# Anony-CFFM/CFFM

Hardware: AMD Instinct MI355X
Metric: training examples/sec, frappe 10-field dim32; embedding-gather %HBM roofline (higher is better)
Workload: dtype f32; 1 GPU; frappe shape: synthetic libfm, 10 fields, 5382 features, inner/outer dim 32, batch 256 per GPU, selu, Adagrad lr 0.05, square_loss (README.md:28); global_batch=256, id_distribution=uniform, tables=replicated, parallelism=single

## Files before the change

cffm_amd/csrc/common.hpp:

```cpp
#pragma once
#include <hip/hip_runtime.h>
#include <stdint.h>

#include "../../include/cffm_hip.h"

#define CFFM_WAVE 64

#ifdef CFFM_PHASE_TIMERS
static __device__ unsigned long long cffm_phase_times[16];
static __device__ unsigned long long cffm_wg_times[2 * 1024];
static __device__ unsigned long long cffm_bwd_times[48];
#define PHASE_MARKB(i, wg) do { if ((wg) == 7 && threadIdx.x == 0) cffm_bwd_times[i] = wall_clock64(); } while (0)
#define PHASE_MARK(i) do { if (blockIdx.x == 7 && threadIdx.x == 0) cffm_phase_times[i] = wall_clock64(); } while (0)
#define PHASE_MARK2(i) do {} while (0)
#define PHASE_MARK3(i) do { if (CL && blockIdx.x == 7 && threadIdx.x == 0) cffm_phase_times[8 + (i)] = wall_clock64(); } while (0)
#else
#define PHASE_MARK(i) do {} while (0)
#define PHASE_MARK2(i) do {} while (0)
#define PHASE_MARK3(i) do {} while (0)
#define PHASE_MARKB(i, wg) do {} while (0)
#endif

typedef float f32x4 __attribute__((ext_vector_type(4)));
__device__ __forceinline__ int fused_c_off(int l, int c0, int c1, int D, int Pp) {
    if (l == 0) return c0;
    int o = c1;
    for (int k = 1; k < l; ++k) { const int S = D >> (k + 1); o += S * S * Pp * 4; }
    return o;
}


#define CFFM_CHECK_LAUNCH()                          \
    do {                                             \
        hipError_t e__ = hipGetLastError();          \
        if (e__ != hipSuccess) return (int)e__;      \
    } while (0)

static inline int ceil_div_i(int64_t a, int64_t b) { return (int)((a + b - 1) / b); }
static inline int ilog2_i(int v) { int r = 0; while ((1 << (r + 1)) <= v) ++r; return r; }
static inline int id_key_bits(int M) {
    int bits = 1;
    while ((1ll << bits) <= (long long)M && bits < 31) ++bits;
    return bits;
}

static constexpr int CFFM_LDS_SHARED_CU = 150 * 1024;
static constexpr int CFFM_LDS_WHOLE_CU = 160 * 1024 - 512;
template <class KernelT>
static inline int set_lds(KernelT k, size_t lds) {
    if (lds > 64 * 1024) {
        hipError_t e = hipFuncSetAttribute((const void*)k, hipFuncAttributeMaxDynamicSharedMemorySize, (int)lds);
        if (e != hipSuccess) return (int)e;
    }
// ... 97 lines not shown
#define CFFM_NSLAB_SMALL 256
static inline int small_slabs(int32_t B) { return B <= 256 ? 256 : (B >= 1024 ? 1024 : (B + 255) / 256 * 256); }
struct SlabRange { int64_t off, len, base; int nslab; };
struct SlabPlan {
    SlabRange r[CFFM_MAX_LAYERS + 3];
    int n;
    int64_t total;
    int head_front, inner, conv0, head_back;
};

static inline bool bwd_top_ok(const cffm_shape_t* s, int32_t B) {
    const int F = s->F, Pp = (F * (F - 1) / 2 + 15) / 16 * 16;
    const int live = ilog2_i(s->D) - 1;
    return Pp <= 64 && B <= 256 && s->inner_conv && s->outer_conv && live >= 2;
}
static inline int bwd_top_first_layer(const cffm_shape_t* s) {
    const int live = ilog2_i(s->D) - 1;
    return live - 2 >= 1 ? live - 2 : 1;
}
static inline int conv_slabs_plain(const cffm_shape_t* s, int32_t B, int l) {
    const int F = s->F, Pp = (F * (F - 1) / 2 + 15) / 16 * 16;
    const int64_t S = s->D >> (l + 1);
    return (Pp <= 64 && (int64_t)B * S * S >= 256 * 64) ? 256 : CFFM_NSLAB;
}
static inline bool conv_pair_slabs_ok(int Pp, int l, int64_t rows, int nslab) {
    return l >= 1 && Pp <= 64 && (rows + nslab - 1) / nslab < 128;
}
static inline bool conv_pair_ok(const cffm_shape_t* s, int32_t B, int l) {
    const int F = s->F, Pp = (F * (F - 1) / 2 + 15) / 16 * 16;
    const int64_t S = s->D >> (l + 1);
    return conv_pair_slabs_ok(Pp, l, (int64_t)B * S * S, conv_slabs_plain(s, B, l));
}
#define CFFM_TOP_SLAB_ROWS 32
static inline bool bwd_fused01_ok(const cffm_shape_t* s, int32_t B) {
    const int F = s->F, Pp = (F * (F - 1) / 2 + 15) / 16 * 16;
    return bwd_top_ok(s, B) && s->D == 32 && Pp <= 48 && B >= 64;
}
static inline bool top_wgrad_deferred(const cffm_shape_t* s, int32_t B) {
    return bwd_top_ok(s, B) && !bwd_fused01_ok(s, B) && conv_pair_ok(s, B, bwd_top_first_layer(s) - 1);
}
static inline int conv_slabs(const cffm_shape_t* s, int32_t B, int l) {
    const int64_t S = s->D >> (l + 1);
    if (bwd_fused01_ok(s, B)) {
        if (l <= 1) return 256;
        const int64_t n = ((int64_t)B * S * S + CFFM_TOP_SLAB_ROWS - 1) / CFFM_TOP_SLAB_ROWS;
        return n < 1 ? 1 : (int)n;
    }
    if (bwd_top_ok(s, B) && l >= bwd_top_first_layer(s)) {
        if (!top_wgrad_deferred(s, B)) return 256;
        const int64_t n = ((int64_t)B * S * S + 63) / 64;
        return n < 1 ? 1 : (n > 256 ? 256 : (int)n);
    }
    return conv_slabs_plain(s, B, l);
}

static inline void make_slab_plan(const cffm_shape_t* s, int32_t B, const cffm_theta_layout_t& tl, SlabPlan* p) {
    int n = 0;
    int64_t base = 0;
    auto add = [&](int64_t off, int64_t end, int nslab) {
        p->r[n].off = off; p->r[n].len = end - off; p->r[n].base = base; p->r[n].nslab = nslab;
        base += (end - off) * nslab;
        return n++;
    };
    const int64_t convs = tl.live > 0 ? tl.conv_w[0] : tl.d1_w;
    p->head_front = add(0, tl.inner_cw, small_slabs(B));
    p->inner = add(tl.inner_cw, convs, small_slabs(B));
    p->conv0 = n;
    for (int l = 0; l < tl.live; ++l)
        add(tl.conv_w[l], l + 1 < tl.live ? tl.conv_w[l + 1] : tl.d1_w, conv_slabs(s, B, l));
// ... 125 lines not shown
```

cffm_amd/csrc/conv.hip:

```cpp
#include <cstdlib>
#include <cstring>

#include "internal.hpp"

#include <type_traits>

#include <stdlib.h>
#include "inner_body.hpp"
#include "head_body.hpp"
#include "sort_body.hpp"

#define KSTEP 32
#define WG_KM 64

__device__ __forceinline__ int64_t xcd_tile(int64_t per_xcd) {
    const int64_t id = blockIdx.x;
    return (id & 7) * per_xcd + (id >> 3);
}
__host__ __device__ static inline int64_t xcd_per(int64_t tiles) { return (tiles + 7) / 8; }

struct RowPos { int b, y, x; };
__device__ __forceinline__ RowPos row_pos(int64_t m, int lgSo) {
    RowPos p;
    const int So = 1 << lgSo;
// ... 1597 lines not shown
        char* smem_i = smem + fa.early_off;
        if (fa.rank_keys) rank_keys_body<NW>(fa.ids, fa.n_rows, b, fa.inner.g.F, fa.inner.g.M, fa.keys_sorted, smem_i);
        PHASE_MARK(0);
        inner_fwd_body<ACT>(fa.inner, b, smem_i, early ? reinterpret_cast<float*>(smem + fa.es_off) : nullptr, fa.inner.g.D + 1, park);
        if (lds_act) lds_barrier(); else __syncthreads();
        PHASE_MARK(1);
        conv0_fact_fwd_body<NT, NW>(fa.conv[0], b, smem, CL(0), early);
        for (int l = 1; l < fa.live; ++l) {
            if (lds_act) lds_barrier(); else __syncthreads();
            PHASE_MARK(1 + l);
            const ConvArgs& ca = fa.conv[l];
            const int64_t rows = 1ll << (2 * ca.lgSo), m_lo = (int64_t)b * rows, m_hi = m_lo + rows;
            if (rows >= 64) {
                for (int64_t m0 = m_lo; m0 < m_hi; m0 += 64) {
                    if (m0 > m_lo) lds_barrier();
                    conv_fwd_taps_body<NT, 4 / G, false, G, ACT>(ca, m0, m_hi, smem, CL(l - 1), CL(l), m_lo);
                }
            } else if (rows >= 32) {
                conv_fwd_taps_body<NT, (G >= 2 ? 1 : 2), false, G, ACT>(ca, m_lo, m_hi, smem, CL(l - 1), CL(l), m_lo);
            } else {
                conv_fwd_taps_body<NT, 1, false, G, ACT>(ca, m_lo, m_hi, smem, CL(l - 1), CL(l), m_lo);
            }
        }
        if (lds_act) lds_barrier(); else __syncthreads();
        PHASE_MARK(1 + fa.live);
        head_fwd_body<NW, ACT>(fa.head, b, smem, lds_act, fa.c0_off, fa.c1_off);
        PHASE_MARK(2 + fa.live);
    }
#ifdef CFFM_PHASE_TIMERS
    if (threadIdx.x == 0) cffm_wg_times[2 * blockIdx.x + 1] = wall_clock64();
#endif
}

template <int NT, int F_, int D_, int NW>
__device__ __forceinline__ void conv0_fact_bwd_body(const DgradArgs& a, float* __restrict__ slabW, float* __restrict__ slabB,
                                                    int64_t slab_stride, char* smem, int wg, int nwg) {
    constexpr int PP = NT * 16, S = 16, NTH = 64 * NW, XQ = 16 / NW;
    const int F = F_ ? F_ : a.F, D = D_ ? D_ : a.D, Dp = D + 1, P = F_ ? F_ * (F_ - 1) / 2 : a.P, F2 = 2 * F;
    const int TP = S * PP + 16;
    float* Wl = reinterpret_cast<float*>(smem);
    float* T = Wl + 4 * PP * PP;
    float* part = T + 2 * F * TP;
    float* dEi = part + NW * 16 * 32;
    float* dEj = dEi + 32 * 16;
    float* bred = dEj + 32 * 16;
    float* rs = bred + NW * PP;
    float* Es = rs + 2 * F;
    const int tid = threadIdx.x, lane = tid & 63, wave = tid >> 6, r = lane & 15, kk = lane >> 4;
    float* sw = slabW + (int64_t)wg * slab_stride;
    float* sb = slabB + (int64_t)wg * slab_stride;
    PHASE_MARKB(12, wg);
    {
        const float4* wsrc = reinterpret_cast<const float4*>(a.W);
        for (int i = tid; i < 4 * PP * PP / 4; i += NTH) reinterpret_cast<float4*>(Wl)[i] = wsrc[i];
        for (int e = tid; e < 4 * (PP - P) * PP; e += NTH) {
            const int tap = e / ((PP - P) * PP), o = e - tap * ((PP - P) * PP);
            sw[(tap * PP + P) * PP + o] = 0.f;
        }
    }
    bool first = true;
    float bacc[NT];
#pragma unroll
    for (int nt = 0; nt < NT; ++nt) bacc[nt] = 0.f;

    for (int b = wg; b < a.B; b += nwg) {
        __syncthreads();
        {
            const float* e = a.Cprev + (int64_t)b * F * D;
            const float invD = 1.f / (float)D;
            for (int i = tid; i < F * D; i += NTH) {
                const int f = fast_div(i, invD), d = i - f * D;
                Es[f * Dp + d] = e[i];
            }
        }
        __syncthreads();
        const float* dCb = a.dC + (int64_t)b * S * S * PP;
        PHASE_MARKB(13, wg);
        for (int u = wave; u < 2 * (F - 1); u += NW) {
            const int i = u % (F - 1), dh = u / (F - 1);
            const int nj = F - 1 - i, K = 2 * nj, base = i * (2 * F - i - 1) / 2;
            f32x4 acc[NT];
#pragma unroll
            for (int nt = 0; nt < NT; ++nt) acc[nt] = (f32x4){0.f, 0.f, 0.f, 0.f};
            for (int k0 = 0; k0 < K; k0 += 4) {
                const int k = k0 + kk;
                const bool ok = k < K;
                const int dw = (ok && k >= nj) ? 1 : 0, jj = ok ? k - dw * nj : 0;
                const float av = ok ? Es[(i + 1 + jj) * Dp + 2 * r + dw] : 0.f;
                const float* wr = Wl + ((dh * 2 + dw) * PP + base + jj) * PP + r;
#pragma unroll
                for (int nt = 0; nt < NT; ++nt) acc[nt] = mfma16(av, ok ? wr[nt * 16] : 0.f, acc[nt]);
            }
            float* tp = T + (dh * F + i) * TP + r;
#pragma unroll
            for (int nt = 0; nt < NT; ++nt)
#pragma unroll
                for (int j = 0; j < 4; ++j) tp[(kk * 4 + j) * PP + nt * 16] = acc[nt][j];
        }
        for (int e = tid; e < 2 * S * PP; e += NTH) {
            const int dh = e / (S * PP), o = e - dh * (S * PP);
            T[(dh * F + F - 1) * TP + o] = 0.f;
        }
        __syncthreads();
        PHASE_MARKB(14, wg);
        {
            f32x4 acc[2] = {(f32x4){0.f, 0.f, 0.f, 0.f}, (f32x4){0.f, 0.f, 0.f, 0.f}};
            float4 av[XQ][NT];
#pragma unroll
            for (int q4 = 0; q4 < XQ; ++q4)
#pragma unroll
                for (int h = 0; h < NT; ++h)
                    av[q4][h] = *reinterpret_cast<const float4*>(dCb + ((int64_t)r * S + wave + NW * q4) * PP + 16 * h + 4 * kk);
#pragma unroll
            for (int q4 = 0; q4 < XQ; ++q4) {
                const int x = wave + NW * q4;
#pragma unroll
                for (int h = 0; h < NT; ++h) {
                    float4 bv[2];
#pragma unroll
                    for (int ct = 0; ct < 2; ++ct) {
                        const int n = ct * 16 + r;
                        bv[ct] = n < F2 ? *reinterpret_cast<const float4*>(T + n * TP + x * PP + 16 * h + 4 * kk)
                                        : make_float4(0.f, 0.f, 0.f, 0.f);
                    }
#pragma unroll
                    for (int ct = 0; ct < 2; ++ct) {
                        acc[ct] = mfma16(av[q4][h].x, bv[ct].x, acc[ct]);
                        acc[ct] = mfma16(av[q4][h].y, bv[ct].y, acc[ct]);
                        acc[ct] = mfma16(av[q4][h].z, bv[ct].z, acc[ct]);
                        acc[ct] = mfma16(av[q4][h].w, bv[ct].w, acc[ct]);
                    }
                }
            }
#pragma unroll
            for (int ct = 0; ct < 2; ++ct)
#pragma unroll
// ... 90 lines not shown
            f32x4 acc[2] = {(f32x4){0.f, 0.f, 0.f, 0.f}, (f32x4){0.f, 0.f, 0.f, 0.f}};
            int ud = 0;
            for (int i = 0; i < F - 1; ++i) ud += 2 * ((2 * (F - 1 - i) + 15) / 16);
            for (int u = (wave + NW - ud % NW) % NW; u < 2 * (F - 1); u += NW) {
                const int i = u % (F - 1), dh = u / (F - 1), base = i * (2 * F - i - 1) / 2;
                const float* ta = T + (dh * F + i) * TP + r * PP + 4 * kk;
                const float* wrow[2];
                bool okc[2];
#pragma unroll
                for (int ct = 0; ct < 2; ++ct) {
                    const int n = ct * 16 + r, dw = n >= F ? 1 : 0, j = n - dw * F;
                    okc[ct] = n < F2 && j > i;
                    wrow[ct] = Wl + ((dh * 2 + dw) * PP + base + (okc[ct] ? j - i - 1 : 0)) * PP + 4 * kk;
                }
#pragma unroll
                for (int h = 0; h < NT; ++h) {
                    const float4 av = *reinterpret_cast<const float4*>(ta + 16 * h);
#pragma unroll
                    for (int ct = 0; ct < 2; ++ct) {
                        const float4 bv = okc[ct] ? *reinterpret_cast<const float4*>(wrow[ct] + 16 * h) : make_float4(0.f, 0.f, 0.f, 0.f);
                        acc[ct] = mfma16(av.x, bv.x, acc[ct]);
                        acc[ct] = mfma16(av.y, bv.y, acc[ct]);
                        acc[ct] = mfma16(av.z, bv.z, acc[ct]);
                        acc[ct] = mfma16(av.w, bv.w, acc[ct]);
                    }
                }
            }
#pragma unroll
            for (int ct = 0; ct < 2; ++ct)
#pragma unroll
                for (int j = 0; j < 4; ++j) part[(wave * 16 + kk * 4 + j) * 32 + ct * 16 + r] = acc[ct][j];
        }
        PHASE_MARKB(18, wg);
        if (tid < 2 * F) {
            const int f = tid % F;
            float sacc = 0.f;
            if (tid < F) { for (int h = 0; h < D; ++h) sacc += Es[f * Dp + h]; }
            else { for (int h = 0; h < D; ++h) sacc += Es[f * Dp + h] * a.dt1[(int64_t)b * a.t1w + h]; }
            rs[tid] = sacc;
        }
        __syncthreads();
        for (int e = tid; e < 16 * 32; e += NTH) {
            float v = part[e];
#pragma unroll
            for (int w = 1; w < NW; ++w) v += part[512 * w + e];
            dEj[(e & 31) * 16 + (e >> 5)] = v;
        }
        __syncthreads();
        PHASE_MARKB(19, wg);
        for (int e = tid; e < F * D; e += NTH) {
            const int f = e / D, h = e - f * D, lo = h & 1, hh = h >> 1;
            float R = 0.f, Q = 0.f;
            for (int j = f + 1; j < F; ++j) R += rs[j];
            for (int i = 0; i < f; ++i) Q += rs[F + i];
            a.dprev[(int64_t)b * F * D + e] = (dEi[(lo * F + f) * 16 + hh] + dEj[(lo * F + f) * 16 + hh])
                                              + a.dt1[(int64_t)b * a.t1w + h] * R + Q;
        }
        first = false;
    }
    PHASE_MARKB(20, wg);
    __syncthreads();
#pragma unroll
    for (int nt = 0; nt < NT; ++nt) {
        float v = bacc[nt];
        v += __shfl_xor(v, 16, 64);
        v += __shfl_xor(v, 32, 64);
        if (kk == 0) bred[wave * PP + nt * 16 + r] = v;
    }
    __syncthreads();
    if (tid < PP) {
        float v = bred[tid];
#pragma unroll
// ... 211 lines not shown
                const int hh = h >> 1, lo = h & 1;
                const int base_f = f * (2 * a.F - f - 1) / 2;
                for (int j = f + 1; j < a.F; ++j) {
                    const int p = base_f + j - f - 1;
                    conv += Ti[((lo * 2 + 0) * PP + p) * So + hh];
                    conv += Ti[((lo * 2 + 1) * PP + p) * So + hh];
                }
                for (int i = 0; i < f; ++i) {
                    const int p = i * (2 * a.F - i - 1) / 2 + f - i - 1;
#pragma unroll
                    for (int hf = 0; hf < HALVES; ++hf) {
                        conv += Tj[((hf * 4 + 0 + lo) * PP + p) * So + hh];
                        conv += Tj[((hf * 4 + 2 + lo) * PP + p) * So + hh];
                    }
                }
            } else {
                const int o = row * Dp + h, st = n_ex * exsz;
                conv = scratch[o];
#pragma unroll
                for (int c = 1; c < NCOPY; ++c) conv += scratch[c * st + o];
            }
            a.dprev[(int64_t)b0 * per + e] = conv + a.dt1[(int64_t)b * a.t1w + h] * R + Q;
        }
    }
}

template <int NT, int RM, bool L0, int HALVES>
__global__ __launch_bounds__(256 * HALVES) void dgrad_taps_kernel(DgradArgs a) {
    extern __shared__ __attribute__((aligned(16))) char smem[];
    dgrad_taps_body<NT, RM, L0, HALVES>(a, blockIdx.x, smem);
}

#define WGT_SUB 256
template <int NT, bool GEN, int HALVES, int ACTC = -1>
__device__ __forceinline__ void wgrad_taps_body(const WgradArgs& a, int slab, int nslab, char* smem, int64_t m_lo_o = -1,
                                                int64_t m_hi_o = -1, int tid_in = -1, bool store = true) {
    const int act = ACTC >= 0 ? ACTC : a.act;
    constexpr int PP = NT * 16, UNR = 4, NTH = 256 * HALVES;
    float* Bs = reinterpret_cast<float*>(smem);
    uint32_t* lut = reinterpret_cast<uint32_t*>(Bs + WGT_SUB * PP);
    float* Es = reinterpret_cast<float*>(lut + (GEN ? PP : 0));
    const int tid = tid_in >= 0 ? tid_in : (int)threadIdx.x, lane = tid & 63, wid = tid >> 6, tap = wid & 3, half = wid >> 2;
    const int r = lane & 15, kk = lane >> 4;
    const int So = 1 << a.lgSo, Sin = 2 * So, P = a.P, Dp = a.D + 1, S2 = So * So, dh = tap >> 1, dw = tap & 1;
    const int n_ex_max = GEN ? WGT_SUB / S2 + 2 : 0;
    f32x4* red = reinterpret_cast<f32x4*>(Es + (GEN ? (n_ex_max * a.F * Dp + 7) / 4 * 4 : 0));
    const int64_t rows_per_slab = ((a.Mtot + nslab - 1) / nslab + 3) / 4 * 4;
    const int64_t m_lo = m_lo_o >= 0 ? m_lo_o : slab * rows_per_slab;
    const int64_t m_hi = m_lo_o >= 0 ? m_hi_o : min(a.Mtot, m_lo + rows_per_slab);

    f32x4 acc[NT][NT];
#pragma unroll
    for (int i = 0; i < NT; ++i)
#pragma unroll
        for (int q = 0; q < NT; ++q) acc[i][q] = (f32x4){0.f, 0.f, 0.f, 0.f};
    float bs[NT];
#pragma unroll
    for (int q = 0; q < NT; ++q) bs[q] = 0.f;
    int fi[NT], fj[NT];
    if (GEN) {
        build_pair_lut(lut, a.F, PP);
        __syncthreads();
#pragma unroll
        for (int i = 0; i < NT; ++i) { const uint32_t ij = lut[i * 16 + r]; fi[i] = (ij & 0xffff) * Dp; fj[i] = (ij >> 16) * Dp; }
    }

    bool done_small = false;
    if constexpr (!GEN && HALVES == 1 && NT <= 4) {
        if (m_hi - m_lo <= 16 * UNR) {
            done_small = true;
            const int dbgw = (a.lgSo == 3 && m_lo_o < 0) ? slab : -1;
            PHASE_MARKB(32, dbgw);
            const int nrow = (int)max((int64_t)0, m_hi - m_lo), nk = (nrow + 3) / 4;
            float av[4][UNR][NT];
#pragma unroll
// ... 107 lines not shown
                    else {
#pragma unroll
                        for (int u = 0; u < UNR; ++u)
#pragma unroll
                            for (int i = 0; i < NT; ++i) av[u][i] = an[u][i];
                    }
                }
            }
        }
    }
    if (HALVES == 2) {
        __syncthreads();
        if (half == 1) {
#pragma unroll
            for (int i = 0; i < NT; ++i)
#pragma unroll
                for (int q = 0; q < NT; ++q) red[(tap * NT * NT + i * NT + q) * 64 + lane] = acc[i][q];
            if (tap == 0) {
#pragma unroll
                for (int q = 0; q < NT; ++q) reinterpret_cast<float*>(red + 4 * NT * NT * 64)[q * 64 + lane] = bs[q];
            }
        }
        __syncthreads();
        if (half == 1) return;
#pragma unroll
        for (int i = 0; i < NT; ++i)
#pragma unroll
            for (int q = 0; q < NT; ++q) acc[i][q] += red[(tap * NT * NT + i * NT + q) * 64 + lane];
        if (tap == 0) {
#pragma unroll
            for (int q = 0; q < NT; ++q) bs[q] += reinterpret_cast<float*>(red + 4 * NT * NT * 64)[q * 64 + lane];
        }
    }
    if (!store) return;
    float* sw = a.slabW + (int64_t)slab * a.slab_stride + (int64_t)tap * PP * PP;
#pragma unroll
    for (int i = 0; i < NT; ++i)
#pragma unroll
        for (int q = 0; q < NT; ++q)
#pragma unroll
            for (int j = 0; j < 4; ++j) sw[(i * 16 + kk * 4 + j) * PP + q * 16 + r] = acc[i][q][j];
    if (tap == 0) {
#pragma unroll
        for (int q = 0; q < NT; ++q) {
            float v = bs[q];
            v += __shfl_xor(v, 16, 64);
            v += __shfl_xor(v, 32, 64);
            if (kk == 0) a.slabB[(int64_t)slab * a.slabB_stride + q * 16 + r] = v;
        }
    }
}

template <int NT, bool GEN, int HALVES>
__global__ __launch_bounds__(256 * HALVES) void wgrad_taps_kernel(WgradArgs a) {
    extern __shared__ __attribute__((aligned(16))) char smem[];
    wgrad_taps_body<NT, GEN, HALVES>(a, blockIdx.x, gridDim.x, smem);
}

struct TopWgrad { WgradArgs w[2]; int n[2]; };
template <int NT, int RM, int ACT = -1>
__global__ __launch_bounds__(256, (NT <= 3 ? 4 : 1)) void conv_bwd_pair_kernel(DgradArgs d, WgradArgs w, int n_d, int n_w, InnerBwdArgs ib, int n_i,
                                                            TopWgrad tw, int xcd_align) {
    extern __shared__ __attribute__((aligned(16))) char smem[];
    int bid = blockIdx.x;
#ifdef CFFM_PHASE_TIMERS
    if (threadIdx.x == 0 && blockIdx.x < 1024) cffm_wg_times[2 * blockIdx.x] = wall_clock64();
#endif
// ... 23 lines not shown
    if (threadIdx.x == 0 && blockIdx.x < 1024) cffm_wg_times[2 * blockIdx.x + 1] = wall_clock64();
#endif
}

struct Conv01Args {
    DgradArgs d0;
    float *slabW0, *slabB0;
    int64_t stride0;
    DgradArgs d1;
    WgradArgs w1, w2, w3;
    int n2, n3;
};

template <int NT, int F_, int D_, int ACT>
__global__ __launch_bounds__(1024) void conv01_bwd_kernel(Conv01Args a) {
    extern __shared__ __attribute__((aligned(16))) char smem[];
    const int b = blockIdx.x, grp = __builtin_amdgcn_readfirstlane((int)(threadIdx.x >> 8)), ltid = threadIdx.x & 255;
    PHASE_MARKB(40, b);
    dgrad_taps_body<NT, 1, false, 4, ACT>(a.d1, b, smem, 0, -1, 4);
    PHASE_MARKB(41, b);
    {
        char* gsm = smem + (size_t)grp * (64 * NT * 16 * 4);
        const WgradArgs& w = grp == 0 ? a.w1 : (grp == 1 ? a.w2 : a.w3);
        const int nsl = grp == 0 ? (int)gridDim.x : (grp == 1 ? a.n2 : a.n3);
        const int slab = grp == 1 ? b - ((int)gridDim.x - a.n2) : b;
        const bool mine = grp < 3 && slab >= 0 && slab < nsl;
        int64_t m_lo = 0, m_hi = 0;
        if (mine) {
            const int64_t per = grp == 0 ? (1ll << (2 * w.lgSo)) : CFFM_TOP_SLAB_ROWS;
            m_lo = (int64_t)slab * per;
            m_hi = min(w.Mtot, m_lo + per);
            if (m_hi < m_lo) m_hi = m_lo;
        }
        wgrad_taps_body<NT, false, 1, ACT>(w, mine ? slab : 0, nsl, gsm, m_lo, m_hi, ltid, mine);
    }
    __syncthreads();
    PHASE_MARKB(42, b);
    conv0_fact_bwd_body<NT, F_, D_, 16>(a.d0, a.slabW0, a.slabB0, a.stride0, smem, b, (int)gridDim.x);
}

struct BwdTopArgs {
    HeadBwdArgs hb;
    DgradArgs d[2];
    WgradArgs w[2];
    int lgSo[2];
    int n_layers;
    int wgrad_here;
    InnerBwdArgs ib;
    int n_inner;
    int n_keys;
    const int32_t* rank_ids;
    unsigned long long* keys_sorted;
    int n_rows;
};

template <int NT, int ACT = -1>
__global__ __launch_bounds__(256) void bwd_top_kernel(BwdTopArgs a) {
    extern __shared__ __attribute__((aligned(16))) char smem[];
    __shared__ float dh1s[CFFM_HEAD_UNITS];
    __shared__ float dt1s[1024];
    __shared__ float red[4];
    const int bid = blockIdx.x;
#ifdef CFFM_PHASE_TIMERS
    if (threadIdx.x == 0) cffm_wg_times[2 * blockIdx.x] = wall_clock64();
#endif
    if (bid < a.n_inner) {
        PHASE_MARKB(36, bid);
        const float L = head_bwd_loss(a.hb, false, red);
        __syncthreads();
        PHASE_MARKB(37, bid);
        if (a.rank_ids != nullptr && a.n_keys == 0) {
// ... 1005 lines not shown

static int launch_conv0_fact_tile_fwd2(const ConvArgs& a, float* wpack, hipStream_t st) {
    constexpr int NW = 8;
    if (wpack == nullptr || a.F > 32 || a.D / 2 > 32) return CFFM_ERR_UNSUPPORTED;
    const int QT = a.Pp / 16, CE = (a.F + 3) / 4, S = a.D / 2;
    float* WA = wpack;
    float4* WE = reinterpret_cast<float4*>(wpack + (int64_t)2 * a.F * QT * 1024);
    hipLaunchKernelGGL(pack_w0_tile_kernel, dim3(2 * a.F * QT), dim3(256), 0, st, a.W, WA, WE, a.F, a.Pp);
    CFFM_CHECK_LAUNCH();
    const size_t lds = (size_t)(8 * CE * (16 * 16 + 16) + (2 * (4 * CE + 1) * (S + 1) + 3) / 4 * 4 + NW * S) * 4 + 16;
    return launch(conv0_fact_tile_fwd2_kernel<NW>, dim3(a.B), dim3(64 * NW), lds, st, a, (const float*)WA);
}

static int launch_conv0_fact_tile_fwd(const ConvArgs& a, hipStream_t st) {
    constexpr int NW = 8;
    const int S = a.D / 2;
    const size_t lds = (size_t)(2 * a.F * (16 * 16 + 16) + a.F * (a.D + 1) + NW * S) * 4 + 16;
    const int64_t grid = (int64_t)a.B * (a.Pp / 16) * (S / 16);
    if (grid > 0x7fffffffll) return CFFM_ERR_UNSUPPORTED;
    return launch(conv0_fact_tile_fwd_kernel<NW>, dim3((unsigned)grid), dim3(64 * NW), lds, st, a);
}

template <int NT>
static int launch_conv0_fact_fwd(const ConvArgs& a, hipStream_t st) {
    return launch(conv0_fact_fwd_kernel<NT>, dim3(a.B), dim3(256), conv0_fact_fwd_lds(NT * 16, a.F, a.D), st, a);
}

static inline bool conv0_fact_ok(const Geo& g) {
    const int S = g.D / 2;
    if (g.Pp > 64 || (S != 16 && S != 32)) return false;
    return conv0_fact_fwd_lds(g.Pp, g.F, g.D) <= CFFM_LDS_SHARED_CU;
}

static inline size_t conv0_fact_bwd_lds(int Pp, int F, int D) {
    const int NW = 16;
    return (size_t)(4 * Pp * Pp + 2 * F * (16 * Pp + 16) + NW * 16 * 32 + 2 * 32 * 16 + NW * Pp + 2 * F + F * (D + 1)) * 4 + 16;
}
static inline bool conv0_fact_bwd_ok(const Geo& g) {
    if (g.Pp > 64 || g.D != 32) return false;
    return conv0_fact_bwd_lds(g.Pp, g.F, g.D) <= CFFM_LDS_WHOLE_CU;
}

template <int NT>
static int launch_conv0_fact_bwd(const DgradArgs& a, float* slabW, float* slabB, int64_t stride, int nsl, hipStream_t st) {
    constexpr int PP = NT * 16;
    constexpr int NW = 16;
    const size_t lds = conv0_fact_bwd_lds(PP, a.F, a.D);
    auto go = [&](auto fv, auto dv) {
        return launch(conv0_fact_bwd_kernel<NT, CV(fv), CV(dv), NW>, dim3(nsl), dim3(64 * NW), lds, st, a, slabW, slabB, stride);
    };
    if constexpr (NT == 3) {
        if (a.F == 10 && a.D == 32) return go(IntC<10>(), IntC<32>());
    } else if constexpr (NT == 1) {
        if (a.F == 6 && a.D == 32) return go(IntC<6>(), IntC<32>());
        if (a.F == 3 && a.D == 32) return go(IntC<3>(), IntC<32>());
    }
    return go(IntC<0>(), IntC<0>());
}

template <int NT, int RM, bool L0, int HALVES>
static int launch_dgrad_taps(const DgradArgs& a, hipStream_t st) {
    constexpr int PP = NT * 16, BM = 16 * RM;
    const int rows_per_wg = L0 ? dgrad0_rows_per_wg(BM, a.lgSo) : BM;
    const int n_ex = L0 ? dgrad0_tile_examples(BM, a.lgSo) : 0;
    const int So = 1 << a.lgSo;
    const bool fast = L0 && RM == 4 && a.lgSo >= 4 && a.lgSo <= 6;
    const size_t scratch = fast ? (size_t)(4 + 4 * HALVES) * PP * So : (size_t)4 * HALVES * n_ex * a.F * (a.D + 1);
    const size_t lds = (L0 ? (size_t)PP + n_ex * a.F * (a.D + 1) + 2 * n_ex * a.F + scratch : 0) * 4 + 16;
    return launch(dgrad_taps_kernel<NT, RM, L0, HALVES>, dim3((unsigned)((a.Mtot + rows_per_wg - 1) / rows_per_wg)), dim3(256 * HALVES),
                  lds, st, a);
// ... 325 lines not shown
    if (check_shape(s) || !s->inner_conv || !s->outer_conv) return false;
    const Geo g = make_geo(s);
    return conv0_tile_fwd_ok(g) && conv0_tile_wgrad_ok(g) && conv0_tile_dgrad2_ok(g) && g.K == g.D && (g.K == 32 || g.K == 64) &&
           cffm_giw_lds_ok();
}

int cffm_conv01_bwd_impl(const StepCtx& c, hipStream_t st) {
    const cffm_shape_t* s = c.s;
    const Geo& g = c.g;
    const int32_t B = c.B;
    if (!bwd_fused01_ok(s, B) || g.live != 4 || !conv0_fact_bwd_ok(g)) return CFFM_ERR_UNSUPPORTED;
    Conv01Args a;
    memset(&a, 0, sizeof(a));
    const WgradArgs w0 = c.wgrad_args(0);
    a.d0 = c.dgrad_args(0);
    a.slabW0 = w0.slabW; a.slabB0 = w0.slabB; a.stride0 = w0.slab_stride;
    a.d1 = c.dgrad_args(1);
    a.w1 = c.wgrad_args(1); a.w2 = c.wgrad_args(2); a.w3 = c.wgrad_args(3);
    a.n2 = c.conv_slab(2).nslab; a.n3 = c.conv_slab(3).nslab;
    if (c.conv_slab(0).nslab != 256 || c.conv_slab(1).nslab != 256 || a.n2 > 256 || a.n3 > 256 ||
        (int64_t)a.n2 * CFFM_TOP_SLAB_ROWS < a.w2.Mtot || (int64_t)a.n3 * CFFM_TOP_SLAB_ROWS < a.w3.Mtot)
        return CFFM_ERR_UNSUPPORTED;
    {
        const void* must[] = {a.d0.dC, a.d0.W, a.d0.Cprev, a.d0.dt1, a.d0.dprev, a.slabW0, a.slabB0, a.d1.dC, a.d1.W, a.d1.Cprev,
                              a.d1.dt1, a.d1.dprev, a.w1.in, a.w1.dC, a.w1.slabW, a.w1.slabB, a.w2.in, a.w2.dC, a.w2.slabW,
                              a.w2.slabB, a.w3.in, a.w3.dC, a.w3.slabW, a.w3.slabB};
        for (const void* q : must)
            if (q == nullptr) return CFFM_ERR_BAD_SHAPE;
        if (a.d0.Mtot <= 0 || a.d1.Mtot <= 0 || a.w1.Mtot <= 0 || a.w2.Mtot <= 0 || a.w3.Mtot <= 0 || a.n2 < 1 || a.n3 < 1 ||
            a.stride0 <= 0 || a.w1.slab_stride <= 0 || a.w2.slab_stride <= 0 || a.w3.slab_stride <= 0)
            return CFFM_ERR_BAD_SHAPE;
    }
    const int NW = 16, PP = g.Pp;
    const size_t lds = conv0_fact_bwd_lds(PP, g.F, g.D);
#define CFFM_C01_LAUNCH(NTV, FV, DV, ACTV)                                                                       \
    do {                                                                                                         \
        int rc = set_lds(conv01_bwd_kernel<NTV, FV, DV, ACTV>, lds);                                             \
        if (rc) return rc;                                                                                       \
        hipLaunchKernelGGL((conv01_bwd_kernel<NTV, FV, DV, ACTV>), dim3(256), dim3(1024), lds, st, a);          \
    } while (0)
    const int nt = PP / 16;
    if (nt == 3 && g.F == 10 && g.act == CFFM_ACT_SELU) CFFM_C01_LAUNCH(3, 10, 32, CFFM_ACT_SELU);
    else if (nt == 3) CFFM_C01_LAUNCH(3, 0, 0, -1);
    else if (nt == 2) CFFM_C01_LAUNCH(2, 0, 0, -1);
    else CFFM_C01_LAUNCH(1, 0, 0, -1);
#undef CFFM_C01_LAUNCH
    CFFM_CHECK_LAUNCH();
    return 0;
}

bool cffm_fwd_all_ok(const cffm_shape_t* s, int32_t B) {
    const Geo g = make_geo(s);
    return s->inner_conv && s->outer_conv && g.Pp <= 64 && conv0_fact_ok(g) && (int64_t)B * s->F <= 4096 && s->F <= RANK_MAXF;
}

template <int NT>
static int launch_fwd_all(const FwdAllArgs& fa, size_t lds, hipStream_t st) {
    constexpr int NW = 8;
    return with_readme_act<NT>(fa.inner.g.act, [&](auto act) {
        constexpr int ACT = decltype(act)::value;
        int rc = set_lds(fwd_all_kernel<NT, NW, ACT>, lds);
        if (rc) return rc;
        hipLaunchKernelGGL((fwd_all_kernel<NT, NW, ACT>), dim3(fa.B < 256 ? fa.B : 256), dim3(64 * NW), lds, st, fa);
        CFFM_CHECK_LAUNCH();
        return 0;
    });
}
// ... 46 lines not shown
```

Baseline: 2.655 million examples/s.

## Overlap conv0 backward prologue with small wgrad work in fused conv01 kernel

In the fused conv01 backward kernel, the fourth wave group now preloads the conv0 weights (via global_load_lds), the embedding row, and computes the T intermediate, row sums and pad zeroing. Meanwhile the other three groups run a new register-staged small wgrad path for the upper layers. The LDS layout is reorganised so a scratch region placed first can hold the wgrad staging without clobbering the preloaded conv0 buffers. The aim is to take the serial conv0 setup off the critical path, at the cost of more LDS, more register pressure, and a stricter eligibility check on LDS size.

```diff
diff --git a/cffm_amd/csrc/common.hpp b/cffm_amd/csrc/common.hpp
--- a/cffm_amd/csrc/common.hpp
+++ b/cffm_amd/csrc/common.hpp
@@ -11,6 +11,7 @@
 static __device__ unsigned long long cffm_wg_times[2 * 1024];
 static __device__ unsigned long long cffm_bwd_times[48];
 #define PHASE_MARKB(i, wg) do { if ((wg) == 7 && threadIdx.x == 0) cffm_bwd_times[i] = wall_clock64(); } while (0)
+#define PHASE_MARKT(i, wg, t) do { if ((wg) == 7 && threadIdx.x == (t)) cffm_bwd_times[i] = wall_clock64(); } while (0)
 #define PHASE_MARK(i) do { if (blockIdx.x == 7 && threadIdx.x == 0) cffm_phase_times[i] = wall_clock64(); } while (0)
 #define PHASE_MARK2(i) do {} while (0)
 #define PHASE_MARK3(i) do { if (CL && blockIdx.x == 7 && threadIdx.x == 0) cffm_phase_times[8 + (i)] = wall_clock64(); } while (0)
@@ -19,6 +20,7 @@
 #define PHASE_MARK2(i) do {} while (0)
 #define PHASE_MARK3(i) do {} while (0)
 #define PHASE_MARKB(i, wg) do {} while (0)
+#define PHASE_MARKT(i, wg, t) do {} while (0)
 #endif
 
 typedef float f32x4 __attribute__((ext_vector_type(4)));
@@ -182,9 +184,14 @@
     return conv_pair_slabs_ok(Pp, l, (int64_t)B * S * S, conv_slabs_plain(s, B, l));
 }
 #define CFFM_TOP_SLAB_ROWS 32
+static inline size_t conv0_fact_bwd_lds(int Pp, int F, int D, bool pre = false) {
+    const int NW = 16, late = NW * 16 * 32 + 2 * 32 * 16 + NW * Pp, scratch = 4 * 64 * Pp;
+    const int front = pre && scratch > late ? scratch : late;
+    return (size_t)(front + 4 * Pp * Pp + 2 * F * (16 * Pp + 16) + 2 * F + F * (D + 1)) * 4 + 16;
+}
 static inline bool bwd_fused01_ok(const cffm_shape_t* s, int32_t B) {
     const int F = s->F, Pp = (F * (F - 1) / 2 + 15) / 16 * 16;
-    return bwd_top_ok(s, B) && s->D == 32 && Pp <= 48 && B >= 64;
+    return bwd_top_ok(s, B) && s->D == 32 && Pp <= 48 && B >= 64 && conv0_fact_bwd_lds(Pp, F, s->D, true) <= (size_t)CFFM_LDS_WHOLE_CU;
 }
 static inline bool top_wgrad_deferred(const cffm_shape_t* s, int32_t B) {
     return bwd_top_ok(s, B) && !bwd_fused01_ok(s, B) && conv_pair_ok(s, B, bwd_top_first_layer(s) - 1);
diff --git a/cffm_amd/csrc/conv.hip b/cffm_amd/csrc/conv.hip
--- a/cffm_amd/csrc/conv.hip
+++ b/cffm_amd/csrc/conv.hip
@@ -1653,31 +1653,140 @@
 #endif
 }
 
-template <int NT, int F_, int D_, int NW>
+template <int NT, int NW, bool PRE>
+struct Conv0BwdLds {
+    float* Wl;
+    float* T;
+    float* part;
+    float* dEi;
+    float* dEj;
+    float* bred;
+    float* rs;
+    float* Es;
+    __device__ __forceinline__ Conv0BwdLds(char* smem, int F) {
+        constexpr int PP = NT * 16, TP = 16 * PP + 16, LATE = NW * 16 * 32 + 2 * 32 * 16 + NW * PP, SCRATCH = 4 * 64 * PP;
+        float* p = reinterpret_cast<float*>(smem);
+        if (PRE) { part = p; p += SCRATCH > LATE ? SCRATCH : LATE; }
+        Wl = p;
+        T = Wl + 4 * PP * PP;
+        p = T + 2 * F * TP;
+        if (!PRE) { part = p; p += LATE; }
+        dEi = part + NW * 16 * 32;
+        dEj = dEi + 32 * 16;
+        bred = dEj + 32 * 16;
+        rs = p;
+        Es = rs + 2 * F;
+    }
+};
+
+template <int NT>
+__device__ __forceinline__ void conv0_fact_T_unit(const float* Wl, const float* Es, float* T, int F, int Dp, int u, int r, int kk) {
+    constexpr int PP = NT * 16, TP = 16 * PP + 16;
+    const int i = u % (F - 1), dh = u / (F - 1);
+    const int nj = F - 1 - i, K = 2 * nj, base = i * (2 * F - i - 1) / 2;
+    f32x4 acc[NT];
+#pragma unroll
+    for (int nt = 0; nt < NT; ++nt) acc[nt] = (f32x4){0.f, 0.f, 0.f, 0.f};
+    for (int k0 = 0; k0 < K; k0 += 4) {
+        const int k = k0 + kk;
+        const bool ok = k < K;
+        const int dw = (ok && k >= nj) ? 1 : 0, jj = ok ? k - dw * nj : 0;
+        const float av = ok ? Es[(i + 1 + jj) * Dp + 2 * r + dw] : 0.f;
+        const float* wr = Wl + ((dh * 2 + dw) * PP + base + jj) * PP + r;
+#pragma unroll
+        for (int nt = 0; nt < NT; ++nt) acc[nt] = mfma16(av, ok ? wr[nt * 16] : 0.f, acc[nt]);
+    }
+    float* tp = T + (dh * F + i) * TP + r;
+#pragma unroll
+    for (int nt = 0; nt < NT; ++nt)
+#pragma unroll
+        for (int j = 0; j < 4; ++j) tp[(kk * 4 + j) * PP + nt * 16] = acc[nt][j];
+}
+
+__device__ __forceinline__ void conv0_fact_row_sum(const DgradArgs& a, const float* Es, float* rs, int F, int D, int Dp, int b, int t) {
+    const int f = t % F;
+    float sacc = 0.f;
+    if (t < F) { for (int h = 0; h < D; ++h) sacc += Es[f * Dp + h]; }
+    else { for (int h = 0; h < D; ++h) sacc += Es[f * Dp + h] * a.dt1[(int64_t)b * a.t1w + h]; }
+    rs[t] = sacc;
+}
+
+__device__ __forceinline__ void conv0_fact_zero_pad_rows(float* sw, int P, int PP, int tid, int nth) {
+    for (int e = tid; e < 4 * (PP - P) * PP; e += nth) {
+        const int tap = e / ((PP - P) * PP), o = e - tap * ((PP - P) * PP);
+        sw[(tap * PP + P) * PP + o] = 0.f;
+    }
+}
+
+template <int NT, int F_, int D_>
+__device__ __forceinline__ void conv0_fact_pre_issue(const DgradArgs& a, float* Wl, int b, int lt, int lw, float (&ev)[2]) {
+    const int F = F_ ? F_ : a.F, D = D_ ? D_ : a.D;
+    if (b < a.B) {
+        const float* e = a.Cprev + (int64_t)b * F * D;
+#pragma unroll
+        for (int it = 0; it < 2; ++it) {
+            const int i = lt + 256 * it;
+            ev[it] = i < F * D ? e[i] : 0.f;
+        }
+        const float4* wsrc = reinterpret_cast<const float4*>(a.W);
+        for (int c = lw; c < 4 * NT * NT; c += 4)
+            __builtin_amdgcn_global_load_lds((const void __attribute__((address_space(1)))*)(wsrc + c * 64 + (lt & 63)),
+                                             (void __attribute__((address_space(3)))*)(Wl + c * 256), 16, 0, 0);
+    }
+}
+template <int NT, int F_, int D_>
+__device__ __forceinline__ void conv0_fact_pre_land(const DgradArgs& a, float* Es, float* T, int b, int lt, const float (&ev)[2]) {
+    constexpr int PP = NT * 16, S = 16, TP = S * PP + 16;
+    const int F = F_ ? F_ : a.F, D = D_ ? D_ : a.D, Dp = D + 1;
+    if (b < a.B) {
+        const float invD = 1.f / (float)D;
+#pragma unroll
+        for (int it = 0; it < 2; ++it) {
+            const int i = lt + 256 * it;
+            if (i < F * D) {
+                const int f = fast_div(i, invD), d = i - f * D;
+                Es[f * Dp + d] = ev[it];
+            }
+        }
+        for (int e = lt; e < 2 * S * PP; e += 256) {
+            const int dh = e / (S * PP), o = e - dh * (S * PP);
+            T[(dh * F + F - 1) * TP + o] = 0.f;
+        }
+        asm volatile("s_waitcnt vmcnt(0)" ::: "memory");
+    }
+}
+template <int NT, int F_, int D_>
+__device__ __forceinline__ void conv0_fact_pre_T(const DgradArgs& a, const Conv0BwdLds<NT, 16, true>& L, float* sw, int b, int lt, int lw) {
+    constexpr int PP = NT * 16;
+    const int F = F_ ? F_ : a.F, D = D_ ? D_ : a.D, Dp = D + 1, P = F_ ? F_ * (F_ - 1) / 2 : a.P;
+    if (b < a.B) {
+        const int lane = lt & 63, r = lane & 15, kk = lane >> 4, NU = 2 * (F - 1);
+        for (int rd = 0; 4 * rd < NU; ++rd) {
+            const int n = 4 * rd + ((rd & 1) ? 3 - lw : lw);
+            if (n < NU) conv0_fact_T_unit<NT>(L.Wl, L.Es, L.T, F, Dp, (n & 1) * (F - 1) + (n >> 1), r, kk);
+        }
+        PHASE_MARKT(45, b, 768);
+        if (lt >= 192 && lt < 192 + 2 * F) conv0_fact_row_sum(a, L.Es, L.rs, F, D, Dp, b, lt - 192);
+        conv0_fact_zero_pad_rows(sw, P, PP, lt, 256);
+    }
+}
+
+template <int NT, int F_, int D_, int NW, bool PRE = false>
 __device__ __forceinline__ void conv0_fact_bwd_body(const DgradArgs& a, float* __restrict__ slabW, float* __restrict__ slabB,
                                                     int64_t slab_stride, char* smem, int wg, int nwg) {
     constexpr int PP = NT * 16, S = 16, NTH = 64 * NW, XQ = 16 / NW;
     const int F = F_ ? F_ : a.F, D = D_ ? D_ : a.D, Dp = D + 1, P = F_ ? F_ * (F_ - 1) / 2 : a.P, F2 = 2 * F;
     const int TP = S * PP + 16;
-    float* Wl = reinterpret_cast<float*>(smem);
-    float* T = Wl + 4 * PP * PP;
-    float* part = T + 2 * F * TP;
-    float* dEi = part + NW * 16 * 32;
-    float* dEj = dEi + 32 * 16;
-    float* bred = dEj + 32 * 16;
-    float* rs = bred + NW * PP;
-    float* Es = rs + 2 * F;
+    const Conv0BwdLds<NT, NW, PRE> L(smem, F);
+    float *Wl = L.Wl, *T = L.T, *part = L.part, *dEi = L.dEi, *dEj = L.dEj, *bred = L.bred, *rs = L.rs, *Es = L.Es;
     const int tid = threadIdx.x, lane = tid & 63, wave = tid >> 6, r = lane & 15, kk = lane >> 4;
     float* sw = slabW + (int64_t)wg * slab_stride;
     float* sb = slabB + (int64_t)wg * slab_stride;
     PHASE_MARKB(12, wg);
-    {
+    if constexpr (!PRE) {
         const float4* wsrc = reinterpret_cast<const float4*>(a.W);
         for (int i = tid; i < 4 * PP * PP / 4; i += NTH) reinterpret_cast<float4*>(Wl)[i] = wsrc[i];
-        for (int e = tid; e < 4 * (PP - P) * PP; e += NTH) {
-            const int tap = e / ((PP - P) * PP), o = e - tap * ((PP - P) * PP);
-            sw[(tap * PP + P) * PP + o] = 0.f;
-        }
+        conv0_fact_zero_pad_rows(sw, P, PP, tid, NTH);
     }
     bool first = true;
     float bacc[NT];
@@ -1685,44 +1794,26 @@
     for (int nt = 0; nt < NT; ++nt) bacc[nt] = 0.f;
 
     for (int b = wg; b < a.B; b += nwg) {
-        __syncthreads();
-        {
-            const float* e = a.Cprev + (int64_t)b * F * D;
-            const float invD = 1.f / (float)D;
-            for (int i = tid; i < F * D; i += NTH) {
-                const int f = fast_div(i, invD), d = i - f * D;
-                Es[f * Dp + d] = e[i];
-            }
-        }
-        __syncthreads();
         const float* dCb = a.dC + (int64_t)b * S * S * PP;
-        PHASE_MARKB(13, wg);
-        for (int u = wave; u < 2 * (F - 1); u += NW) {
-            const int i = u % (F - 1), dh = u / (F - 1);
-            const int nj = F - 1 - i, K = 2 * nj, base = i * (2 * F - i - 1) / 2;
-            f32x4 acc[NT];
-#pragma unroll
-            for (int nt = 0; nt < NT; ++nt) acc[nt] = (f32x4){0.f, 0.f, 0.f, 0.f};
-            for (int k0 = 0; k0 < K; k0 += 4) {
-                const int k = k0 + kk;
-                const bool ok = k < K;
-                const int dw = (ok && k >= nj) ? 1 : 0, jj = ok ? k - dw * nj : 0;
-                const float av = ok ? Es[(i + 1 + jj) * Dp + 2 * r + dw] : 0.f;
-                const float* wr = Wl + ((dh * 2 + dw) * PP + base + jj) * PP + r;
-#pragma unroll
-                for (int nt = 0; nt < NT; ++nt) acc[nt] = mfma16(av, ok ? wr[nt * 16] : 0.f, acc[nt]);
-            }
-            float* tp = T + (dh * F + i) * TP + r;
-#pragma unroll
-            for (int nt = 0; nt < NT; ++nt)
-#pragma unroll
-                for (int j = 0; j < 4; ++j) tp[(kk * 4 + j) * PP + nt * 16] = acc[nt][j];
-        }
-        for (int e = tid; e < 2 * S * PP; e += NTH) {
-            const int dh = e / (S * PP), o = e - dh * (S * PP);
-            T[(dh * F + F - 1) * TP + o] = 0.f;
-        }
-        __syncthreads();
+        if constexpr (!PRE) {
+            __syncthreads();
+            {
+                const float* e = a.Cprev + (int64_t)b * F * D;
+                const float invD = 1.f / (float)D;
+                for (int i = tid; i < F * D; i += NTH) {
+                    const int f = fast_div(i, invD), d = i - f * D;
+                    Es[f * Dp + d] = e[i];
+                }
+            }
+            __syncthreads();
+            PHASE_MARKB(13, wg);
+            for (int u = wave; u < 2 * (F - 1); u += NW) conv0_fact_T_unit<NT>(Wl, Es, T, F, Dp, u, r, kk);
+            for (int e = tid; e < 2 * S * PP; e += NTH) {
+                const int dh = e / (S * PP), o = e - dh * (S * PP);
+                T[(dh * F + F - 1) * TP + o] = 0.f;
+            }
+            __syncthreads();
+        }
         PHASE_MARKB(14, wg);
         {
             f32x4 acc[2] = {(f32x4){0.f, 0.f, 0.f, 0.f}, (f32x4){0.f, 0.f, 0.f, 0.f}};
@@ -1879,12 +1970,8 @@
                 for (int j = 0; j < 4; ++j) part[(wave * 16 + kk * 4 + j) * 32 + ct * 16 + r] = acc[ct][j];
         }
         PHASE_MARKB(18, wg);
-        if (tid < 2 * F) {
-            const int f = tid % F;
-            float sacc = 0.f;
-            if (tid < F) { for (int h = 0; h < D; ++h) sacc += Es[f * Dp + h]; }
-            else { for (int h = 0; h < D; ++h) sacc += Es[f * Dp + h] * a.dt1[(int64_t)b * a.t1w + h]; }
-            rs[tid] = sacc;
+        if constexpr (!PRE) {
+            if (tid < 2 * F) conv0_fact_row_sum(a, Es, rs, F, D, Dp, b, tid);
         }
         __syncthreads();
         for (int e = tid; e < 16 * 32; e += NTH) {
@@ -2162,15 +2249,96 @@
 }
 
 #define WGT_SUB 256
+template <int NT>
+struct WgradSmall {
+    int nrow, nk;
+    float av[4][4][NT];
+};
+template <int NT>
+__device__ __forceinline__ void wgrad_small_issue(const WgradArgs& a, int64_t m_lo, int64_t m_hi, int tid, WgradSmall<NT>& s) {
+    constexpr int PP = NT * 16, UNR = 4;
+    const int lane = tid & 63, tap = (tid >> 6) & 3, r = lane & 15, kk = lane >> 4;
+    const int So = 1 << a.lgSo, Sin = 2 * So, dh = tap >> 1, dw = tap & 1;
+    s.nrow = (int)max((int64_t)0, m_hi - m_lo);
+    s.nk = (s.nrow + 3) / 4;
+#pragma unroll
+    for (int g = 0; g < 4; ++g)
+        if (g * UNR < s.nk) {
+#pragma unroll
+            for (int u = 0; u < UNR; ++u) {
+                int64_t m = m_lo + 4 * (g * UNR + u) + kk;
+                if (g * UNR + u >= s.nk || m >= a.Mtot) m = a.Mtot - 1;
+                const RowPos rp = row_pos(m, a.lgSo);
+                const float* arow = a.in + (((int64_t)rp.b * Sin + 2 * rp.y + dh) * Sin + 2 * rp.x + dw) * PP + r;
+#pragma unroll
+                for (int i = 0; i < NT; ++i) s.av[g][u][i] = arow[16 * i];
+            }
+        }
+}
+template <int NT>
+__device__ __forceinline__ void wgrad_small_stage(const WgradArgs& a, int64_t m_lo, float* Bs, int tid, const WgradSmall<NT>& s) {
+    constexpr int PP = NT * 16, NTH = 256;
+    const float4* src = reinterpret_cast<const float4*>(a.dC + m_lo * PP);
+    for (int e = tid; e < s.nrow * (PP / 4); e += NTH) reinterpret_cast<float4*>(Bs)[e] = src[e];
+    for (int e = s.nrow * (PP / 4) + tid; e < 4 * s.nk * (PP / 4); e += NTH)
+        reinterpret_cast<float4*>(Bs)[e] = make_float4(0.f, 0.f, 0.f, 0.f);
+}
+template <int NT>
+__device__ __forceinline__ void wgrad_small_mfma(const float* Bs, int act, int tid, const WgradSmall<NT>& s, f32x4 (&acc)[NT][NT],
+                                                 float (&bs)[NT]) {
+    constexpr int PP = NT * 16, UNR = 4;
+    const int lane = tid & 63, r = lane & 15, kk = lane >> 4;
+#pragma unroll
+    for (int g = 0; g < 4; ++g)
+        if (g * UNR < s.nk) {
+#pragma unroll
+            for (int u = 0; u < UNR; ++u)
+                if (g * UNR + u < s.nk) {
+                    float bv[NT];
+#pragma unroll
+                    for (int q = 0; q < NT; ++q) bv[q] = Bs[(4 * (g * UNR + u) + kk) * PP + q * 16 + r];
+#pragma unroll
+                    for (int q = 0; q < NT; ++q) bs[q] += bv[q];
+#pragma unroll
+                    for (int i = 0; i < NT; ++i) {
+                        const float x = act_pos(s.av[g][u][i], act);
+#pragma unroll
+                        for (int q = 0; q < NT; ++q) acc[i][q] = mfma16(x, bv[q], acc[i][q]);
+                    }
+                }
+        }
+}
+template <int NT>
+__device__ __forceinline__ void wgrad_slab_store(const WgradArgs& a, int slab, int tid, const f32x4 (&acc)[NT][NT], const float (&bs)[NT]) {
+    constexpr int PP = NT * 16;
+    const int lane = tid & 63, tap = (tid >> 6) & 3, r = lane & 15, kk = lane >> 4;
+    float* sw = a.slabW + (int64_t)slab * a.slab_stride + (int64_t)tap * PP * PP;
+#pragma unroll
+    for (int i = 0; i < NT; ++i)
+#pragma unroll
+        for (int q = 0; q < NT; ++q)
+#pragma unroll
+            for (int j = 0; j < 4; ++j) sw[(i * 16 + kk * 4 + j) * PP + q * 16 + r] = acc[i][q][j];
+    if (tap == 0) {
+#pragma unroll
+        for (int q = 0; q < NT; ++q) {
+            float v = bs[q];
+            v += __shfl_xor(v, 16, 64);
+            v += __shfl_xor(v, 32, 64);
+            if (kk == 0) a.slabB[(int64_t)slab * a.slabB_stride + q * 16 + r] = v;
+        }
+    }
+}
+
 template <int NT, bool GEN, int HALVES, int ACTC = -1>
 __device__ __forceinline__ void wgrad_taps_body(const WgradArgs& a, int slab, int nslab, char* smem, int64_t m_lo_o = -1,
-                                                int64_t m_hi_o = -1, int tid_in = -1, bool store = true) {
+                                                int64_t m_hi_o = -1) {
     const int act = ACTC >= 0 ? ACTC : a.act;
     constexpr int PP = NT * 16, UNR = 4, NTH = 256 * HALVES;
     float* Bs = reinterpret_cast<float*>(smem);
     uint32_t* lut = reinterpret_cast<uint32_t*>(Bs + WGT_SUB * PP);
     float* Es = reinterpret_cast<float*>(lut + (GEN ? PP : 0));
-    const int tid = tid_in >= 0 ? tid_in : (int)threadIdx.x, lane = tid & 63, wid = tid >> 6, tap = wid & 3, half = wid >> 2;
+    const int tid = threadIdx.x, lane = tid & 63, wid = tid >> 6, tap = wid & 3, half = wid >> 2;
     const int r = lane & 15, kk = lane >> 4;
     const int So = 1 << a.lgSo, Sin = 2 * So, P = a.P, Dp = a.D + 1, S2 = So * So, dh = tap >> 1, dw = tap & 1;
     const int n_ex_max = GEN ? WGT_SUB / S2 + 2 : 0;
@@ -2344,7 +2512,6 @@
             for (int q = 0; q < NT; ++q) bs[q] += reinterpret_cast<float*>(red + 4 * NT * NT * 64)[q * 64 + lane];
         }
     }
-    if (!store) return;
     float* sw = a.slabW + (int64_t)slab * a.slab_stride + (int64_t)tap * PP * PP;
 #pragma unroll
     for (int i = 0; i < NT; ++i)
@@ -2434,11 +2601,39 @@
             m_hi = min(w.Mtot, m_lo + per);
             if (m_hi < m_lo) m_hi = m_lo;
         }
-        wgrad_taps_body<NT, false, 1, ACT>(w, mine ? slab : 0, nsl, gsm, m_lo, m_hi, ltid, mine);
+        const int lw = __builtin_amdgcn_readfirstlane(ltid >> 6);
+        const Conv0BwdLds<NT, 16, true> L(smem, F_ ? F_ : a.d0.F);
+        float* Bs = reinterpret_cast<float*>(gsm);
+        const int act = ACT >= 0 ? ACT : w.act;
+        WgradSmall<NT> sm;
+        f32x4 acc[NT][NT];
+        float bs[NT], ev[2] = {0.f, 0.f};
+#pragma unroll
+        for (int i = 0; i < NT; ++i)
+#pragma unroll
+            for (int q = 0; q < NT; ++q) acc[i][q] = (f32x4){0.f, 0.f, 0.f, 0.f};
+#pragma unroll
+        for (int q = 0; q < NT; ++q) bs[q] = 0.f;
+        PHASE_MARKT(43, b, 768);
+        if (grp < 3) wgrad_small_issue<NT>(w, m_lo, m_hi, ltid, sm);
+        else conv0_fact_pre_issue<NT, F_, D_>(a.d0, L.Wl, b, ltid, lw, ev);
+        __syncthreads();
+        if (grp < 3) wgrad_small_stage<NT>(w, m_lo, Bs, ltid, sm);
+        else conv0_fact_pre_land<NT, F_, D_>(a.d0, L.Es, L.T, b, ltid, ev);
+        __syncthreads();
+        PHASE_MARKT(44, b, 768);
+        if (grp < 3) {
+            wgrad_small_mfma<NT>(Bs, act, ltid, sm, acc, bs);
+            if (mine) wgrad_slab_store<NT>(w, slab, ltid, acc, bs);
+        } else {
+            conv0_fact_pre_T<NT, F_, D_>(a.d0, L, a.slabW0 + (int64_t)b * a.stride0, b, ltid, lw);
+        }
+        PHASE_MARKB(47, b);
+        PHASE_MARKT(46, b, 768);
     }
     __syncthreads();
     PHASE_MARKB(42, b);
-    conv0_fact_bwd_body<NT, F_, D_, 16>(a.d0, a.slabW0, a.slabB0, a.stride0, smem, b, (int)gridDim.x);
+    conv0_fact_bwd_body<NT, F_, D_, 16, true>(a.d0, a.slabW0, a.slabB0, a.stride0, smem, b, (int)gridDim.x);
 }
 
 struct BwdTopArgs {
@@ -3510,10 +3705,6 @@
     return conv0_fact_fwd_lds(g.Pp, g.F, g.D) <= CFFM_LDS_SHARED_CU;
 }
 
-static inline size_t conv0_fact_bwd_lds(int Pp, int F, int D) {
-    const int NW = 16;
-    return (size_t)(4 * Pp * Pp + 2 * F * (16 * Pp + 16) + NW * 16 * 32 + 2 * 32 * 16 + NW * Pp + 2 * F + F * (D + 1)) * 4 + 16;
-}
 static inline bool conv0_fact_bwd_ok(const Geo& g) {
     if (g.Pp > 64 || g.D != 32) return false;
     return conv0_fact_bwd_lds(g.Pp, g.F, g.D) <= CFFM_LDS_WHOLE_CU;
@@ -3905,7 +4096,8 @@
             return CFFM_ERR_BAD_SHAPE;
     }
     const int NW = 16, PP = g.Pp;
-    const size_t lds = conv0_fact_bwd_lds(PP, g.F, g.D);
+    const size_t lds = conv0_fact_bwd_lds(PP, g.F, g.D, true);
+    if (lds > (size_t)CFFM_LDS_WHOLE_CU || g.F * g.D > 512) return CFFM_ERR_UNSUPPORTED;
 #define CFFM_C01_LAUNCH(NTV, FV, DV, ACTV)                                                                       \
     do {                                                                                                         \
         int rc = set_lds(conv01_bwd_kernel<NTV, FV, DV, ACTV>, lds);                                             \
```

Measured after the change: 2.656 million examples/s (median of 3 runs). Within noise of the previous version (+0.1%).
